# leggedrobotics/raisimLib

Measured on AMD Instinct MI355X. Metric: env-steps/sec, 4096 ANYmal-C envs flat terrain dt=0.0025, higher is better.
Workload: dtype f32

## Files before the change

include/rsb_ext.h:

```cpp
#ifndef RSB_EXT_H_
#define RSB_EXT_H_

#include "rsb.h"

#ifdef __cplusplus
extern "C" {
#endif

int rsb_set_solver_stagnation_exit(rsb_world* w, int window, double factor);
int rsb_set_solver_friction_lag(rsb_world* w, int freeze_after, int refine, double settle_tol);
int rsb_set_solver_multi_contact(rsb_world* w, int depth, int light_passes, int freeze_after, int stall_window);
int rsb_set_solver_anderson(rsb_world* w, int first_sweep, double clip);
#define RSB_SLIP_ENERGY 0
#define RSB_SLIP_COULOMB 1
int rsb_set_slip_rule(rsb_world* w, int rule);

int rsb_set_early_termination(rsb_world* w, int on);
int rsb_set_solver_warm_start(rsb_world* w, int on);

int rsb_set_lanes_per_env(rsb_world* w, int lanes);
int rsb_get_lanes_per_env(const rsb_world* w);

int rsb_set_heightmap_contacts(rsb_world* w, int per_primitive, double min_angle_deg);
int rsb_set_capsule_contacts(rsb_world* w, int on);
// ... 16 lines not shown
int rsb_model_lds_bytes(const rsb_model* m, int kmax, int self_collision, int lanes_per_env);
int rsb_model_delassus_layout(const rsb_model* m, int kmax, int self_collision, int* out4);
int rsb_model_up_quads(const rsb_model* m, int* table, int capacity);

#define RSB_SPEC_OFF 0
#define RSB_SPEC_CACHED 1
#define RSB_SPEC_COMPILE 2
int rsb_set_specialization(rsb_world* w, int mode);
int rsb_specialization_status(const rsb_world* w, long long* specialized_launches, long long* generic_launches);
const char* rsb_spec_dir(void);
int rsb_spec_compile(const char* manifest_line);
int rsb_spec_file_name(const char* manifest_line, char* out, int capacity);


int rsb_last_kernel_ms(rsb_world* w, float* ms);
int rsb_enable_timing(rsb_world* w, int on);
int rsb_set_timing_stride(rsb_world* w, int stride);
int rsb_read_kernel_ms(rsb_world* w, float* ms, int n);

int rsb_debug_select_env(rsb_world* w, int env);
int rsb_debug_read_contact_problem(rsb_world* w, int* nc, float* G, float* c, float* lam);
int rsb_debug_phase_cycles(rsb_world* w, int enable, long long* out16);
int rsb_debug_wave_profile(rsb_world* w, long long* out, int n_blocks);


#ifdef __cplusplus
}
#endif

#endif
```

raisimlib_amd/_capi.py:

```python
import ctypes as C
import os

RSB_MAX_BODIES = 64
RSB_MAX_DOF = 6 + RSB_MAX_BODIES - 1
RSB_MAX_COLLISIONS = 64
RSB_MAX_CONTACTS = 16
RSB_NAME_LEN = 48

RSB_HOST, RSB_DEVICE = 0, 1
RSB_CONTACT_SELF_A, RSB_CONTACT_SELF_B, RSB_CONTACT_SECOND, RSB_CONTACT_CAPSULE = 0x10000, 0x20000, 0x40000, 0x80000
RSB_FORCE_AND_TORQUE, RSB_PD_PLUS_FEEDFORWARD_TORQUE = 0, 1
(RSB_F_GC, RSB_F_GV, RSB_F_PTARGET, RSB_F_DTARGET, RSB_F_TAU_FF, RSB_F_CONTACT_COUNT, RSB_F_CONTACTS,
 RSB_F_FLAGS, RSB_F_GENERALIZED_FORCE) = range(9)

_B, _S = RSB_MAX_BODIES, RSB_MAX_COLLISIONS


class ModelBlob(C.Structure):
    _fields_ = [
        ("nb", C.c_int32), ("nq", C.c_int32), ("nv", C.c_int32), ("ncol", C.c_int32), ("depth", C.c_int32),
        ("fixed_base", C.c_int32),
        ("parent", C.c_int32 * _B), ("level", C.c_int32 * _B), ("jtype", C.c_int32 * _B),
        ("axis", (C.c_double * 3) * _B), ("ptree", (C.c_double * 3) * _B), ("rtree", (C.c_double * 9) * _B),
        ("mass", C.c_double * _B), ("com", (C.c_double * 3) * _B), ("inertia", (C.c_double * 6) * _B),
# ... 209 lines not shown
    "rsb_last_kernel_ms": (_I, [_VP, C.POINTER(C.c_float)]),
    "rsb_enable_timing": (_I, [_VP, _I]),
    "rsb_set_timing_stride": (_I, [_VP, _I]),
    "rsb_read_kernel_ms": (_I, [_VP, _FP, _I]),
    "rsb_control_step": (_I, [_VP, _FP, _FP, _I, _FP, _FP, _I, _FP, _I, _FP, _FP, _I]),
    "rsb_control_steps": (_I, [_VP, _I, _FP, _I, C.c_longlong, _I, _FP, C.c_longlong, _FP, _I, _FP, _I, _FP, _FP, _I, _VP, C.c_longlong]),
    "rsb_set_step_residency": (_I, [_VP, _I]),
    "rsb_step_residency_enabled": (_I, [_VP]),
    "rsb_step_residency_status": (_I, [_VP, _I]),
    "rsb_step_residency_launches": (C.c_longlong, [_VP]),
    "rsb_debug_resident_full_writes": (_I, [_VP, _I]),
    "rsb_model_lds_bytes": (_I, [_VP, _I, _I, _I]),
    "rsb_model_up_quads": (_I, [_VP, _VP, _I]),
    "rsb_model_delassus_layout": (_I, [_VP, _I, _I, _VP]),
    "rsb_set_specialization": (_I, [_VP, _I]),
    "rsb_specialization_status": (_I, [_VP, C.POINTER(C.c_longlong), C.POINTER(C.c_longlong)]),
    "rsb_spec_dir": (C.c_char_p, []),
    "rsb_spec_compile": (_I, [C.c_char_p]),
    "rsb_spec_file_name": (_I, [C.c_char_p, C.c_char_p, _I]),
    "rsb_debug_view_profile": (_I, [_VP, C.POINTER(C.c_longlong), _I]),
    "rsb_debug_select_env": (_I, [_VP, _I]),
    "rsb_debug_phase_cycles": (_I, [_VP, _I, _FP]),
    "rsb_debug_wave_profile": (_I, [_VP, _FP, _I]),
    "rsb_debug_read_contact_problem": (_I, [_VP, C.POINTER(C.c_int), _FP, _FP, _FP]),
}

_lib = None


def lib():
    global _lib
    if _lib is None:
        if not os.path.exists(LIB_PATH):
            raise RuntimeError(
                f"{LIB_PATH} is missing: build it with `python -c 'import __graft_entry__ as g; g.build()'` "
                "(hipcc --offload-arch=gfx950). raisimlib_amd has no CPU fallback.")
        L = C.CDLL(LIB_PATH, mode=C.RTLD_GLOBAL)
        for name, (res, args) in PROTOTYPES.items():
            fn = getattr(L, name)
            fn.restype, fn.argtypes = res, args
        _lib = L
    return _lib


class RsbError(RuntimeError):
    pass
# ... 7 lines not shown
```

raisimlib_amd/csrc/rsb_world.hip:

```cpp
#include <dlfcn.h>
#include <hip/hip_runtime.h>

#include <algorithm>
#include <cmath>
#include <cstdio>
#include <cstdlib>
#include <chrono>
#include <cstring>
#include <memory>
#include <string>
#include <vector>

#include "query_kernel.h"
#include "rsb.h"
#include "rsb_internal.h"
#include "step_launch.h"
#include "env_task.h"
#include "step_types.h"


#include "rsb_world.h"
#include "rsb_spec.h"

namespace rsbw {
// ... 1639 lines not shown
  if (c) std::memcpy(c, buf.data() + 1 + n3 * n3, sizeof(float) * n3);
  if (lam) std::memcpy(lam, buf.data() + 1 + n3 * n3 + n3, sizeof(float) * n3);
  return RSB_OK;
}

int rsb_debug_phase_cycles(rsb_world* w, int enable, long long* out16) {
  if (!w) return RSB_E_INVALID;
  HIP_TRY(hipSetDevice(w->device));
  const size_t nprof = 16 + 16 * (size_t)w->N;
  if (enable && !w->d_prof) { HIP_TRY(hipMalloc(&w->d_prof, nprof * sizeof(long long))); HIP_TRY(hipMemset(w->d_prof, 0, nprof * sizeof(long long))); }
  if (out16 && w->d_prof) {
    HIP_TRY(hipMemcpyAsync(out16, w->d_prof, 16 * sizeof(long long), hipMemcpyDeviceToHost, stream_of(w)));
    HIP_TRY(hipStreamSynchronize(stream_of(w)));
  }
  if (!enable && w->d_prof) { HIP_TRY(hipStreamSynchronize(stream_of(w))); HIP_TRY(hipFree(w->d_prof)); w->d_prof = nullptr; }
  return RSB_OK;
}

int rsb_debug_wave_profile(rsb_world* w, long long* out, int n_blocks) {
  if (!w || !out || !w->d_prof || n_blocks > w->N) return RSB_E_INVALID;
  HIP_TRY(hipSetDevice(w->device));
  HIP_TRY(hipMemcpyAsync(out, w->d_prof + 16, 16 * (size_t)n_blocks * sizeof(long long), hipMemcpyDeviceToHost, stream_of(w)));
  HIP_TRY(hipStreamSynchronize(stream_of(w)));
  return RSB_OK;
}

int rsb_enable_timing(rsb_world* w, int on) {
  if (!w || on < 0) return RSB_E_INVALID;
  HIP_TRY(hipSetDevice(w->device));
  for (hipEvent_t e : w->ring0) (void)hipEventDestroy(e);
  for (hipEvent_t e : w->ring1) (void)hipEventDestroy(e);
  w->ring0.clear(); w->ring1.clear(); w->ring_next = w->ring_count = 0;
  w->launch_index = 0;
  w->timing = on != 0;
  if (on > 1) {
    w->ring0.resize(on); w->ring1.resize(on);
    for (int i = 0; i < on; ++i) { HIP_TRY(hipEventCreate(&w->ring0[i])); HIP_TRY(hipEventCreate(&w->ring1[i])); }
  }
  return RSB_OK;
}
int rsb_set_timing_stride(rsb_world* w, int stride) {
  if (!w || stride < 1) return RSB_E_INVALID;
  w->timing_stride = stride; w->launch_index = 0;
  return RSB_OK;
}
int rsb_read_kernel_ms(rsb_world* w, float* ms, int n) {
// ... 23 lines not shown
```

raisimlib_amd/csrc/step_kernel.h:

```cpp
#pragma once

#include <hip/hip_runtime.h>
#include <stdint.h>

#include <type_traits>

#include "env_task.h"
#include "rsb_types.h"
#include "step_types.h"
#include "step_spec.h"
#include "step_math.h"
#include "step_terrain.h"
#include "step_slip.h"
#include "step_slip_pk.h"
#include "stage_bodies.h"

#ifndef RSB_X_RES_RING
#define RSB_X_RES_RING 0
#endif
#if defined(RSB_I_CL) && ((RSB_I_CL) & 64)
#define RSB_RESIDENT 1
#else
#define RSB_RESIDENT 0
#endif
// ... 257 lines not shown
  for (int sub = 0; sub < nsub; ++sub) {
    RSB_STAMP(0)
    RSB_ARGS(ab);
    tsq = 0.f;
#include "step_phase_tree_down.inc"
#include "step_phase_collision.inc"
#include "step_phase_tree_up.inc"
    iters_used = 0;
    float wlam[6] = {0.f, 0.f, 0.f, 0.f, 0.f, 0.f};
    if (ncw > 0) {
      RSB_ARGS(aw);
      const float erp = RSB_DIM_F32(ERP, aw.erp);
#include "step_phase_columns.inc"
#include "step_phase_delassus.inc"
#include "step_phase_solver.inc"
    } else if (has_warm) {
      for (int i = s; i < nwarm; i += LPE) WARM[i] = 0.f;
    }
    RSB_STAMP(6)

#include "step_phase_update.inc"
  }

  if (PROF && a.prof && lane == 0) { long long* P = a.prof + 16 + 16 * (long long)blk; P[8] = t_setup; P[9] = t_newt; P[10] = t_epi; P[11] = t_rule; P[12] = t_exch; P[13] = t_end; P[14] = t_start - t_entry; P[15] = t_mag; P[0] = clock64() - t_start; P[1] = t_gs; P[2] = p_iters; P[3] = p_ncw; P[4] = p_search; P[5] = p_newton; P[6] = p_solves; P[7] = t_srch; }
#if RSB_LEAN_SEAM
  if (ls_ok && cs + 1 < ncs) {
#include "step_phase_seam_lean.inc"
  } else {
    seam_refill = true;
    asm volatile("; rsb generic seam begin");
#endif
#include "step_phase_epilogue.inc"
#if RSB_LEAN_SEAM
    asm volatile("; rsb generic seam end");
  }
#endif
#if RSB_RESIDENT
  }
#endif
}

}
```

raisimlib_amd/csrc/step_phase_prologue.inc:

```
  const float* env_heights = a.heights;
  if (a.hm_index && a.terrain_type == 1) env_heights += (size_t)a.hm_index[env] * a.hm_xs * a.hm_ys;
  float rq[2], rpt[2], ru[2], rdt[2], rtf[2], ract[2] = {0.f, 0.f}, ramean[2] = {0.f, 0.f}, wrec[8];
  if constexpr (PIPE) {
    if (a.pipe_wait_on) {
      int spins = 0;
      long long t0 = 0;
      const long long t_in = a.pipe_stats ? wall_clock64() : 0;
      while (__builtin_amdgcn_readfirstlane(__hip_atomic_load(a.pipe_wait_ptr + (size_t)blk * a.pipe_stride, __ATOMIC_RELAXED, __HIP_MEMORY_SCOPE_AGENT)) - a.pipe_wait < 0) {
        if (__builtin_amdgcn_readfirstlane(__hip_atomic_load(a.pipe_err, __ATOMIC_RELAXED, __HIP_MEMORY_SCOPE_AGENT)) != 0) return;
        __builtin_amdgcn_s_sleep(8);
        if ((++spins & 255) == 0) {
          const long long now = wall_clock64();
          if (t0 == 0) t0 = now;
          else if (now - t0 > a.pipe_timeout) {
            if (lane == 0 && atomicCAS(a.pipe_err, 0, 2 ) == 0) __hip_atomic_store(a.pipe_err_host, 2, __ATOMIC_RELAXED, __HIP_MEMORY_SCOPE_SYSTEM);
            return;
          }
        }
      }
      if (a.pipe_stats && lane == 0) {
        __hip_atomic_fetch_add(a.pipe_stats, (unsigned long long)(wall_clock64() - t_in), __ATOMIC_RELAXED, __HIP_MEMORY_SCOPE_AGENT);
        if (spins > 0) __hip_atomic_fetch_add(a.pipe_stats + 1, 1ull, __ATOMIC_RELAXED, __HIP_MEMORY_SCOPE_AGENT);
      }
    }
// ... 53 lines not shown
    if (i < nv) { U[i] = (fixed_base && i < 6) ? 0.f : ru[k]; DTG[i] = rdt[k]; TF[i] = rtf[k]; }
  }
  __syncthreads();
  const bool isbody = s >= 1 && s < nb;
  const int bb = isbody ? s : 0;
  const int mylev = isbody ? (PARLV[bb] >> 8) : -1;
  const int mypar = max((PARLV[bb] & 0xff) - 1, 0);
  const int mykid = KIDX[bb];
  const int nkid0 = KIDX[0] >> 16;
  const int kid_first = KIDS[mykid & 0xffff];
  int kid0s[4];
  RSB_UNROLL for (int i = 0; i < 4; ++i) kid0s[i] = __builtin_amdgcn_readfirstlane(KIDS[i]);
  const int max_kid = RSB_DIM(MAX_KID, a.max_kid);
  if (a.warm && s < a.kmax) {
    const int col = __float_as_int(wrec[6]) - 1;
    if (col >= 0 && col < ncol) { RSB_UNROLL for (int i = 0; i < 6; ++i) WARM[6 * col + i] = wrec[i]; }
  }
  int flag = 0, iters_used = 0, nc = 0;
  int nc_real = 0;
  int nselfc = 0;
  bool dead = false;
  int nc_dead = 0;
  long long t_start = 0, t_gs = 0, t_srch = 0, t_setup = 0, t_newt = 0, t_epi = 0, t_rule = 0, t_exch = 0, t_end = 0; int p_iters = 0, p_ncw = 0, p_search = 0, p_newton = 0, p_solves = 0;
  if (PROF && a.prof) t_start = clock64();
  const bool pfine = PROF && a.prof && a.prof_fine;
  long long t_prev = 0, t_mag = 0;
  auto lap = [&](long long& acc) { if (PROF && pfine) { const long long t = clock64(); acc += t - t_prev; t_prev = t; } };
  float pbx = 0.f, pby = 0.f, pbz = 0.f;
  const float dt = a.dt;
  const int nsub = RSB_DIM(NSUB, a.nsub), kmax = RSB_DIM(KMAX, a.kmax);
  const bool has_warm = RSB_DIM(HAS_WARM, a.warm != nullptr);
  __syncthreads();

  float tsq = 0.f;
```

raisimlib_amd/csrc/step_phase_solver.inc:

```
      if (PROF && a.dbg && env == a.dbg_env && env_valid && s == 0) {
        const int n3 = 3 * nc_real;
        a.dbg[0] = (float)nc_real;
        for (int i = 0; i < n3; ++i)
          for (int j = 0; j < n3; ++j)
            a.dbg[1 + i * n3 + j] = GROWS ? G[(i / 3) * GRP + kGBlock * (j / 3) + g_block_off(i % 3, j % 3)] : !TRI ? G[i * GS + 4 * (j / 3) + (j % 3)]
                                          : (i / 3 >= j / 3 ? G[tri_off(i / 3, j / 3) + 4 * (i % 3) + (j % 3)] : G[tri_off(j / 3, i / 3) + 4 * (j % 3) + (i % 3)]);
        for (int i = 0; i < n3; ++i) a.dbg[1 + n3 * n3 + i] = CV[i];
      }
      long long t_gs0 = 0, tz0 = 0; if (PROF && a.prof) t_gs0 = clock64();
      {
        const bool isc = s < nc;
        float Gii[9], Ginv[12], v[3], lam[3] = {0.f, 0.f, 0.f};
        const float* Gmine = GROWS ? G + GRP * min(s, KMAX - 1) : G + 3 * min(s, KMAX - 1) * GS;
        RSB_UNROLL for (int q2 = 0; q2 < 9; ++q2) Gii[q2] = 0.f;
        RSB_UNROLL for (int q2 = 0; q2 < 12; ++q2) Ginv[q2] = 0.f;
        v[0] = v[1] = v[2] = 0.f;
#if RSB_FLAT_CLASS
        asm volatile("; rsb setup begin");
#endif
#if RSB_FLAT_SETUP_HEAD
        static_assert(GROWS && !TRI, "flat set-up: the row-block layout of the quadruped classes");
        const int sq = min(s, KMAX - 1);
        float fq0[5][4], fq1[5][4], fq2[5], fc4[4], fc8[4];
        {
// ... 92 lines not shown
        int wcount = 0;

        int gpos = 0, gdw = 1;
        bool light = false;
        bool multi = false;
        int sw_env = stall_window > 0 ? stall_window : -1;
        {
          static_for<0, KMAX / 4>([&](auto bc) {
            constexpr int j0 = 4 * decltype(bc)::value;
            if (j0 < ncw) {
              static_for<0, 4>([&](auto kc2) {
                constexpr int j = j0 + decltype(kc2)::value;
                const int gj = __builtin_amdgcn_update_dpp(0, gidc, 0x150 + j, 0xf, 0xf, true);
                gpos += ((gj == gidc) & (j < s)) ? 1 : 0;
              });
            }
          });
          const int gd = row_max_i32(isc ? gpos + 1 : 1);
          multi = (RSB_DIM(MULTI_DEPTH, ag.multi_depth) > 0) & (gd >= RSB_DIM(MULTI_DEPTH, ag.multi_depth));
          light = multi & (RSB_DIM(MULTI_LIGHT, ag.multi_light) != 0);
          sw_env = multi ? (RSB_DIM(MULTI_SW, ag.multi_stall_window) > 0 ? RSB_DIM(MULTI_SW, ag.multi_stall_window) : -1) : sw_env;
          gdw = env_groups_max<LPE>(gd);
        }
#ifndef RSB_X_AA8
#define RSB_X_AA8 0
#endif
        constexpr bool AA = TRI || RSB_X_AA8;
        const int aa_first = AA ? ag.anderson : 0;
        const float aa_clip = ag.anderson_clip;
        const bool aa_on = AA && multi && aa_first > 0;
        float aa_x[3] = {0.f, 0.f, 0.f}, aa_g[3] = {0.f, 0.f, 0.f}, aa_r[3] = {0.f, 0.f, 0.f};

        const int sm = min(s, KMAX - 1);
        auto coupling = [&](int k, float (&g)[3][4]) {
          if constexpr (TRI) {
            const bool tr = k > sm;
            const float* bp = G + tri_off(tr ? k : sm, tr ? sm : k);
            float t[3][4];
            RSB_UNROLL for (int rr = 0; rr < 3; ++rr) ld4(bp + 4 * rr, t[rr]);
            RSB_UNROLL for (int rr = 0; rr < 3; ++rr) {
              RSB_UNROLL for (int cc = 0; cc < 3; ++cc) g[rr][cc] = tr ? t[cc][rr] : t[rr][cc];
              g[rr][3] = 0.f;
            }
          } else if constexpr (GROWS) {
            float t[3][3];
            gblk_load(Gmine + kGBlock * k, t);
// ... 67 lines not shown
          auto one = [&](auto jc) {
            constexpr int j = decltype(jc)::value;
            float l0[3] = {x[0], x[1], x[2]};
            row_bcast_n<j, 3>(l0);
            if constexpr (PK && j < NPK) {
              float2v acc = {v[0], v[1]};
              RSB_UNROLL for (int cc = 0; cc < 3; ++cc) acc = __builtin_elementwise_fma(gp[j][cc], float2v{l0[cc], l0[cc]}, acc);
              v[0] = acc.x; v[1] = acc.y;
              v[2] = fmaf(gr[j][2], l0[2], fmaf(gr[j][1], l0[1], fmaf(gr[j][0], l0[0], v[2])));
            } else if constexpr (PK && !TRI && j < 8) {
              float gt[3][4];
              coupling(j, gt);
              RSB_UNROLL for (int rr = 0; rr < 3; ++rr)
                v[rr] = fmaf(gt[rr][2], l0[2], fmaf(gt[rr][1], l0[1], fmaf(gt[rr][0], l0[0], v[rr])));
            } else {
              const float (&gj)[3][4] = PK ? gbuf[(j / 4) & 1][j & 3] : (j < 4 ? g0[PK ? 0 : (j & 3)] : (j < 8 ? g1[PK ? 0 : (j & 3)] : (j < 12 ? g2[(KMAX > 8 && !PK ? j : 0) & 3] : gbuf[(j / 4) & 1][j & 3])));
              RSB_UNROLL for (int rr = 0; rr < 3; ++rr)
                v[rr] = fmaf(gj[rr][2], l0[2], fmaf(gj[rr][1], l0[1], fmaf(gj[rr][0], l0[0], v[rr])));
            }
            emax = fmaxf(emax, fmaxf(fabsf(l0[0]), fmaxf(fabsf(l0[1]), fabsf(l0[2]))));
          };
          static_for<0, 5>(one);
          {
            if (ncw > 5) {
              one(std::integral_constant<int, 5>{});
              if (ncw > 6) {
                one(std::integral_constant<int, 6>{});
                if (ncw > 7) {
                  one(std::integral_constant<int, 7>{});
                  static_for<2, KMAX / 4>([&](auto bc) {
                    constexpr int b = decltype(bc)::value;
                    if (4 * b < ncw) {
                      if constexpr (b >= 3 || (PK && 4 * b >= NPK)) load_block(bc);
                      static_for<4 * b, 4 * b + 4>(one);
                    }
                  });
                }
              }
            }
          }
        };

        if (has_warm) {
#if RSB_FLAT_SETUP_HEAD
          {
            const bool wok = isc && mycol < ncol;
            lam[0] = wok ? fwr[0] : 0.f; lam[1] = wok ? fwr[1] : 0.f; lam[2] = wok ? fwr[2] : 0.f;
// ... 33 lines not shown
          row_bcast_dyn_n<KMAX, 13>(c12, j);
          SlipCoef kb;
          kb.a0 = c12[0]; kb.a1 = c12[1]; kb.a2 = c12[2]; kb.n00 = c12[3]; kb.n01 = c12[4]; kb.n02 = c12[5];
          kb.n10 = c12[6]; kb.n11 = c12[7]; kb.n12 = c12[8]; kb.vn = c12[9]; kb.ls0 = c12[10]; kb.ls1 = c12[11];
          float dxy[2];
          slip_search<LPE, COUL>(kb, c12[12], section_rounds, s, el, c16, s16, DIR16, dxy);
          if (take) { sdx = dxy[0]; sdy = dxy[1]; sdst = 1; }
        };

#if !defined(RSB_X_ALIGN_SWEEP) && defined(RSB_SPECIALIZED)
#define RSB_X_ALIGN_SWEEP 0
#endif
#ifndef RSB_X_ALIGN_SWEEP
#define RSB_X_ALIGN_SWEEP 7
#endif
#ifndef RSB_X_ALIGN_SWEEP_TRI
#define RSB_X_ALIGN_SWEEP_TRI 7
#endif
        asm volatile(".p2align 5");
        static_for<0, (TRI ? RSB_X_ALIGN_SWEEP_TRI : RSB_X_ALIGN_SWEEP)>([&](auto) { asm volatile("s_nop 0"); });
#if RSB_PK_CLASS
        asm volatile("; rsb sweep begin");
#endif
        for (int it = 0; it < max_iter; ++it) {
          const bool lag = multi ? (multi_fa > 0 && it >= multi_fa) : (freeze_after > 0 && it >= freeze_after);
          float err = 0.f;
          float dl_last[3] = {0.f, 0.f, 0.f};
          if constexpr (AA) { aa_x[0] = lam[0]; aa_x[1] = lam[1]; aa_x[2] = lam[2]; }
          for (int kp = 0; kp < gdw; ++kp) {
            const bool mine = isc & !done & (gpos == kp);
            if (PROF && a.prof) ++p_solves;
            float ls[3];
#if RSB_PK_SOLVE
            const f32x2 ls01 = pk_stick(gip, f32x2{v[0], v[1]}, v[2], f32x2{lam[0], lam[1]});
            ls[0] = ls01.x; ls[1] = ls01.y;
            ls[2] = fmaf(-Ginv[8], v[2], fmaf(-Ginv[7], v[1], fmaf(-Ginv[6], v[0], lam[2])));
#else
            RSB_UNROLL for (int rr = 0; rr < 3; ++rr)
              ls[rr] = fmaf(-Ginv[3 * rr + 2], v[2], fmaf(-Ginv[3 * rr + 1], v[1], fmaf(-Ginv[3 * rr], v[0], lam[rr])));
#endif
            const float vexn = fmaf(-Gii[8], lam[2], fmaf(-Gii[7], lam[1], fmaf(-Gii[6], lam[0], v[2])));
            const bool open = vexn > 0.f;
            const bool stick = (!open) & (ls[2] >= 0.f) & (fmaf(ls[1], ls[1], ls[0] * ls[0]) <= (mu2 * ls[2]) * ls[2]);
            const bool slip = (!open) & (!stick);
            const bool usable = (sdst == 1) & (fmaf(sc.a2, sdy, fmaf(sc.a1, sdx, sc.a0)) >= kDenFreeze * sc.a0);
            const bool keep = lag & usable;
            const bool refr = isc & !done & (light ? (kp == 0) : (gpos == kp));
            bool need = refr & slip & !keep;
            const bool lost = mine & slip & !refr & !usable;
            lap(t_rule);
#ifdef RSB_X_NO_NEWTON
            if (false) {
#else
            if (__any(need | lost)) {
#endif
              SlipCoef kc;
              kc = sc;
#if RSB_PK_SOLVE
              SlipCoefPk kp;
              pk_coef(kp, sc.a0, sc.a1, sc.a2, gcp[2], mg1, mg2, pk_vex(gcp, f32x2{v[0], v[1]}, f32x2{lam[0], lam[1]}, lam[2]), vexn, ls01);
              kc = slip_unpack(kp);
#else
              {
                const float vex0 = v[0] - (Gii[0] * lam[0] + Gii[1] * lam[1] + Gii[2] * lam[2]);
                const float vex1 = v[1] - (Gii[3] * lam[0] + Gii[4] * lam[1] + Gii[5] * lam[2]);
                kc.n00 = sc.a0 * vex0 - vexn * Gii[2]; kc.n01 = sc.a1 * vex0 - vexn * sc.n01; kc.n02 = sc.a2 * vex0 - vexn * sc.n02;
                kc.n10 = sc.a0 * vex1 - vexn * Gii[5]; kc.n11 = sc.a1 * vex1 - vexn * sc.n11; kc.n12 = sc.a2 * vex1 - vexn * sc.n12;
                kc.vn = vexn; kc.ls0 = ls[0]; kc.ls1 = ls[1];
              }
#endif
              if (PROF && a.prof) ++p_newton;
              float nx, ny, dstep;
#if RSB_PK_SOLVE
              bool ok = slip_newton_pk(kp, mu, sdx, sdy, nx, ny, dstep) & need & (sdst != 0) & (refine != 0);
#else
              bool ok = slip_newton<COUL>(kc, mu, sdx, sdy, nx, ny, dstep) & need & (sdst != 0) & (refine != 0);
#endif
#ifdef RSB_X_STAMP_BASIN
              lap(t_newt);
#endif
#ifdef RSB_X_NO_BASIN
              if (false) {
#else
              if (it == 0 && !COUL) {
#endif
                const bool chk = ok & (sdst == 3);
                if (__any(chk)) {
                  float ebest;
#ifndef RSB_X_SERIAL_BASIN
                  if (ncw <= 4) {
                    const int row = lane & ~15, q = lane & 3;
                    const int from_owner = (row | ((lane >> 2) & 3)) << 2, from_quad = (row | ((lane & 3) << 2)) << 2;
                    float c13[13] = {kc.a0, kc.a1, kc.a2, kc.n00, kc.n01, kc.n02, kc.n10, kc.n11, kc.n12, kc.vn, kc.ls0, kc.ls1, mu};
                    RSB_UNROLL for (int i = 0; i < 13; ++i) c13[i] = __int_as_float(__builtin_amdgcn_ds_bpermute(from_owner, __float_as_int(c13[i])));
                    SlipCoef kq;
                    kq.a0 = c13[0]; kq.a1 = c13[1]; kq.a2 = c13[2]; kq.n00 = c13[3]; kq.n01 = c13[4]; kq.n02 = c13[5];
                    kq.n10 = c13[6]; kq.n11 = c13[7]; kq.n12 = c13[8]; kq.vn = c13[9]; kq.ls0 = c13[10]; kq.ls1 = c13[11];
                    float e = __int_as_float(0x7f800000);
                    const bool swp = (q & 1) != 0;
                    const unsigned sgx = ((q + 1) & 2) ? 0x80000000u : 0u, sgy = (q & 2) ? 0x80000000u : 0u;
                    RSB_UNROLL for (int i = 0; i < 4; ++i) {
                      const float x = __uint_as_float(__float_as_uint(swp ? kSin16[i] : kCos16[i]) ^ sgx);
                      const float y = __uint_as_float(__float_as_uint(swp ? kCos16[i] : kSin16[i]) ^ sgy);
                      e = fminf(e, slip_E(kq, c13[12], x, y));
                    }
                    e = fminf(e, __int_as_float(__builtin_amdgcn_update_dpp(0, __float_as_int(e), 0xB1, 0xf, 0xf, true)));
                    e = fminf(e, __int_as_float(__builtin_amdgcn_update_dpp(0, __float_as_int(e), 0x4E, 0xf, 0xf, true)));
                    ebest = __int_as_float(__builtin_amdgcn_ds_bpermute(from_quad, __float_as_int(e)));
#ifdef RSB_X_BASIN_VERIFY
                    {
                      float e2 = slip_E(kc, mu, 1.0f, 0.0f);
                      RSB_UNROLL for (int i = 1; i < 16; ++i) e2 = fminf(e2, slip_E(kc, mu, kCos16[i], kSin16[i]));
                      if (chk && __float_as_int(e2) != __float_as_int(ebest)) flag |= 16;
                    }
#endif
                  } else
#endif
                  {
                    SlipCoef ks = kc;
#ifndef RSB_X_SERIAL_BASIN
                    asm volatile("" : "+v"(ks.a0), "+v"(ks.a1), "+v"(ks.a2));
#endif
                    ebest = slip_E(ks, mu, 1.0f, 0.0f);
                    RSB_UNROLL for (int i = 1; i < 16; ++i) ebest = fminf(ebest, slip_E(ks, mu, kCos16[i], kSin16[i]));
                  }
                  ok = ok & !(chk & !(slip_E(kc, mu, nx, ny) <= ebest));
                }
              }
#ifdef RSB_X_STAMP_BASIN
              lap(t_mag);
#endif
              sdx = ok ? nx : sdx; sdy = ok ? ny : sdy; sdst = ok ? 1 : sdst;
              need = (need & !ok) | lost;
              if (__any(need)) {
                for (int j = 0; j < ncw; ++j)
                  if (__any(need && s == j)) search_row(j, kc, need && s == j);
              }
              lap(t_newt);
            }
            const float den = fmaf(sc.a2, sdy, fmaf(sc.a1, sdx, sc.a0));
            const float lnn = -vexn * __builtin_amdgcn_rcpf(fmaxf(den, kDenMin * sc.a0));
            const float ltn = mu * lnn;
            float ln[3];
            float dl[3];
#if RSB_PK_SOLVE
            {
              const f32x2 lt = pk_splat(ltn) * f32x2{sdx, sdy};
              ln[0] = slip ? lt.x : (stick ? ls[0] : 0.f);
              ln[1] = slip ? lt.y : (stick ? ls[1] : 0.f);
              ln[2] = slip ? lnn : (stick ? ls[2] : 0.f);
              const f32x2 l01 = f32x2{lam[0], lam[1]}, df = pk_splat(alpha) * (f32x2{ln[0], ln[1]} - l01);
              dl[0] = mine ? df.x : 0.f; dl[1] = mine ? df.y : 0.f;
              dl[2] = mine ? alpha * (ln[2] - lam[2]) : 0.f;
              const f32x2 ln01 = l01 + f32x2{dl[0], dl[1]};
              lam[0] = ln01.x; lam[1] = ln01.y; lam[2] += dl[2];
            }
#else
            ln[0] = slip ? ltn * sdx : (stick ? ls[0] : 0.f);
            ln[1] = slip ? ltn * sdy : (stick ? ls[1] : 0.f);
            ln[2] = slip ? lnn : (stick ? ls[2] : 0.f);
            RSB_UNROLL for (int rr = 0; rr < 3; ++rr) {
              dl[rr] = mine ? alpha * (ln[rr] - lam[rr]) : 0.f;
              lam[rr] += dl[rr];
            }
#endif
            lap(t_mag);
            if constexpr (AA) {
              if (kp + 1 < gdw) exchange(dl, err);
              else { dl_last[0] = dl[0]; dl_last[1] = dl[1]; dl_last[2] = dl[2]; }
            } else {
              exchange(dl, err);
            }
            lap(t_exch);
          }
          if constexpr (AA)
            err = fmaxf(err, row_max_f32(fmaxf(fabsf(dl_last[0]), fmaxf(fabsf(dl_last[1]), fabsf(dl_last[2])))));
          if (it == 0) sdst = (sdst == 3) ? 0 : sdst;
          const float scale = row_max_f32(isc ? lam[2] : 0.f);
          {
            const bool live = !done;
            iters_used += live ? 1 : 0;
            alpha = fmaxf(alpha * alpha_decay, alpha_min);
            const float denom = scale + kLambdaFloor;
            const bool conv_now = live & (err <= threshold * denom);
            const float rel = err * __builtin_amdgcn_rcpf(denom);
            const bool cont = live & !conv_now;
            const bool better = cont & (rel < best_rel);
            best_rel = better ? rel : best_rel;
            RSB_UNROLL for (int rr = 0; rr < 3; ++rr) lam_best[rr] = better ? lam[rr] : lam_best[rr];
            best_cur = cont ? fminf(best_cur, rel) : best_cur;
            wcount += cont ? 1 : 0;
            const bool wfull = cont & (wcount == sw_env);
            const bool stalled = wfull & (best_cur > stall_factor * best_prev);
            best_prev = wfull ? best_cur : best_prev;
            best_cur = wfull ? 3e38f : best_cur;
            wcount = wfull ? 0 : wcount;
            converged |= conv_now;
            done |= conv_now | stalled;
          }
          lap(t_epi);
          if (!__any(!done)) break;
          if constexpr (AA) {
            if (__any(aa_on & !done)) {
              float rr[3], num = 0.f, den = 0.f;
              RSB_UNROLL for (int q2 = 0; q2 < 3; ++q2) {
                rr[q2] = lam[q2] - aa_x[q2];
                const float dr = rr[q2] - aa_r[q2];
                num = fmaf(rr[q2], dr, num); den = fmaf(dr, dr, den);
              }
              num = row_sum_f32(isc ? num : 0.f); den = row_sum_f32(isc ? den : 0.f);
              if constexpr (LPE > 16) {
                num = __shfl(num, (lane & ~(LPE - 1)) | (lane & 15)); den = __shfl(den, (lane & ~(LPE - 1)) | (lane & 15));
              }
              const bool use = aa_on & !done & (it >= 1) & (it + 1 >= aa_first) & (den > 1e-30f);
              float gam = use ? num / den : 0.f;
              gam = (fabsf(gam) <= aa_clip) ? gam : 0.f;
              float xn[3], dl[3];
              RSB_UNROLL for (int q2 = 0; q2 < 3; ++q2) { xn[q2] = fmaf(-gam, lam[q2] - aa_g[q2], lam[q2]); aa_g[q2] = lam[q2]; aa_r[q2] = rr[q2]; }
              const float t2 = fmaf(xn[1], xn[1], xn[0] * xn[0]), lim = mu * xn[2];
              const float sh = (t2 > lim * lim) ? lim * __builtin_amdgcn_rsqf(t2) : 1.f;
              const bool off = xn[2] <= 0.f;
              xn[0] = off ? 0.f : xn[0] * sh; xn[1] = off ? 0.f : xn[1] * sh; xn[2] = off ? 0.f : xn[2];
              const bool app = isc & (gam != 0.f);
              RSB_UNROLL for (int q2 = 0; q2 < 3; ++q2) { dl[q2] = app ? xn[q2] - lam[q2] : 0.f; lam[q2] += dl[q2]; dl_last[q2] += dl[q2]; }
// ... 142 lines not shown
```

raisimlib_amd/csrc/step_slip_pk.h:

```cpp
#pragma once

#include "step_slip.h"

#define RSB_PK_NO_CONTRACT _Pragma("clang fp contract(off)")

namespace rsbk {

typedef float f32x2 __attribute__((ext_vector_type(2)));

__device__ __forceinline__ f32x2 pk_splat(float a) { return f32x2{a, a}; }
__device__ __forceinline__ f32x2 pk_fma(f32x2 a, f32x2 b, f32x2 c) { return __builtin_elementwise_fma(a, b, c); }
__device__ __forceinline__ f32x2 pk_swap(f32x2 a) { return f32x2{a.y, a.x}; }

struct SlipCoefPk { float a0, a1, a2, vn; f32x2 n0, n1, n2, ls; };

__device__ __forceinline__ SlipCoef slip_unpack(const SlipCoefPk& k) {
  SlipCoef s;
  s.a0 = k.a0; s.a1 = k.a1; s.a2 = k.a2; s.vn = k.vn;
  s.n00 = k.n0.x; s.n10 = k.n0.y; s.n01 = k.n1.x; s.n11 = k.n1.y; s.n02 = k.n2.x; s.n12 = k.n2.y;
  s.ls0 = k.ls.x; s.ls1 = k.ls.y;
  return s;
}

__device__ __forceinline__ f32x2 pk_stick(const f32x2 (&gi)[3], f32x2 v01, float v2, f32x2 lam01) { RSB_PK_NO_CONTRACT
// ... 24 lines not shown

__device__ __forceinline__ float slip_newton_step_pk(const SlipCoefPk& k, float x0, float y0, float den, float& hp) { RSB_PK_NO_CONTRACT
  const f32x2 xx = pk_splat(x0), yy = pk_splat(y0), ym = f32x2{-y0, y0};
  const float mdp = __builtin_fmaf(k.a2, x0, -(k.a1 * y0));
  const f32x2 N = pk_fma(yy, k.n2, pk_fma(xx, k.n1, k.n0));
  const f32x2 dN = pk_fma(xx, k.n2, -(yy * k.n1));
  const f32x2 PQ = pk_fma(xx, pk_swap(N), ym * N);
  const f32x2 AB = pk_fma(xx, pk_swap(dN), ym * dN);
  const float h = __builtin_fmaf(den, PQ.x, -(mdp * PQ.y));
  hp = __builtin_fmaf(-mdp, AB.y, __builtin_fmaf(den, AB.x, -(k.a0 * PQ.y)));
  return -h * __builtin_amdgcn_rcpf(hp);
}

__device__ __forceinline__ f32x2 slip_rotate_pk(f32x2 d0, float d) { RSB_PK_NO_CONTRACT
  const float d2 = d * d;
  const float c = __builtin_fmaf(-d2, __builtin_fmaf(-d2, 1.0f / 24.0f, 0.5f), 1.0f);
  const float t = __builtin_fmaf(-d2, __builtin_fmaf(-d2, 1.0f / 120.0f, 1.0f / 6.0f), 1.0f);
  const f32x2 sn = f32x2{-d, d} * pk_splat(t);
  const f32x2 xy = pk_fma(d0, pk_splat(c), pk_swap(d0) * sn);
  const float inv = __builtin_amdgcn_rsqf(__builtin_fmaf(xy.x, xy.x, xy.y * xy.y));
  return xy * pk_splat(inv);
}

__device__ __forceinline__ bool slip_newton_pk(const SlipCoefPk& k, float mu, float x0, float y0, float& x1, float& y1, float& step) { RSB_PK_NO_CONTRACT
  const float den0 = pk_den(k, x0, y0);
  float hp;
  const float d = slip_newton_step_pk(k, x0, y0, den0, hp);
  const f32x2 xy = slip_rotate_pk(f32x2{x0, y0}, d);
  const float den1 = pk_den(k, xy.x, xy.y);
  bool ok = (den0 > kDenNewton * k.a0) && (hp > 0.f) && (fabsf(d) <= 0.25f) && (den1 > kDenNewton * k.a0);
  if (__any(ok && fabsf(d) > 0.02f)) ok = ok && (fabsf(d) <= 0.02f || slip_E_pk(k, mu, xy.x, xy.y, den1) <= slip_E_pk(k, mu, x0, y0, den0));
  x1 = xy.x; y1 = xy.y; step = d;
  return ok;
}

}
```

raisimlib_amd/csrc/step_spec.h:

```cpp
#pragma once

#define RSB_SPEC_FIELDS(X)                                                                                                              \
  X(NB, a.nb) X(NQ, a.nq) X(NV, a.nv) X(DEPTH, a.depth) X(NCOL, a.ncol) X(MAX_KID, a.max_kid) X(FIXED_BASE, (a.fixed_base != 0))      \
  X(N_SELF, a.n_self) X(NSUB, a.nsub) X(KMAX, a.kmax) X(HAS_WARM, (a.warm != nullptr)) X(TERRAIN, a.terrain_type)                      \
  X(EARLY_TERM, (a.early_term != 0)) X(SECTION_ROUNDS, a.section_rounds) X(STALL_WINDOW, a.stall_window) X(FREEZE_AFTER, a.freeze_after) \
  X(REFINE, a.refine) X(MULTI_FA, a.multi_freeze_after) X(MULTI_DEPTH, a.multi_depth) X(MULTI_LIGHT, a.multi_light)                    \
  X(MULTI_SW, a.multi_stall_window) X(CHAIN, (a.chain != 0)) X(MODEL_PITCH, a.L.model_pitch) \
  X(UP_QUADS, (a.chain == 2)) \
  X(MU, rsbk::spec_bits(a.mu)) X(ERP, rsbk::spec_bits(a.erp)) X(ALPHA_INIT, rsbk::spec_bits(a.alpha_init)) X(ALPHA_MIN, rsbk::spec_bits(a.alpha_min)) \
  X(ALPHA_DECAY, rsbk::spec_bits(a.alpha_decay)) X(THRESHOLD, rsbk::spec_bits(a.threshold)) X(STALL_FACTOR, rsbk::spec_bits(a.stall_factor)) \
  X(MAX_ITER, a.max_iter)

#ifdef RSB_SPECIALIZED
#define RSB_DIM(NAME, expr) (RSB_SPEC_##NAME)
#else
#define RSB_DIM(NAME, expr) (expr)
#endif

namespace rsbk {
constexpr int spec_bits(float f) { return __builtin_bit_cast(int, f); }
constexpr float spec_f32(int bits) { return __builtin_bit_cast(float, bits); }
}
#if defined(RSB_SPECIALIZED) && !defined(RSB_X_NO_SPEC_CONSTS)
#define RSB_SPEC_CONSTS 1
// ... 89 lines not shown
#if RSB_FLAT_SETUP && RSB_FLAT_SCATTER && !defined(RSB_X_NO_FLAT_SETUP_END)
#define RSB_FLAT_SETUP_END 1
#else
#define RSB_FLAT_SETUP_END 0
#endif

#if RSB_FLAT_SETUP && (RSB_I_KMAX) == 8 && RSB_SPEC_UP_QUADS && !defined(RSB_X_NO_FLAT_DELASSUS)
#define RSB_FLAT_DELASSUS 1
#else
#define RSB_FLAT_DELASSUS 0
#endif

#if defined(RSB_SPECIALIZED) && defined(RSB_I_LPE) && (RSB_I_LPE) == 16 && (RSB_I_KMAX) <= 8 && !((RSB_I_CL) & 32)
#define RSB_PK_CLASS 1
#else
#define RSB_PK_CLASS 0
#endif
#if RSB_PK_CLASS && !defined(RSB_X_NO_PK_SOLVE)
#define RSB_PK_SOLVE 1
#else
#define RSB_PK_SOLVE 0
#endif

namespace rsbk {
#define RSB_SPEC_COUNT_ONE(NAME, expr) +1
constexpr int kSpecFields = 0 RSB_SPEC_FIELDS(RSB_SPEC_COUNT_ONE);
#undef RSB_SPEC_COUNT_ONE
}
```

raisimlib_amd/world.py:

```python
import ctypes as C
import os

import numpy as np

from . import _capi
from ._capi import (RSB_DEVICE, RSB_F_GENERALIZED_FORCE, RSB_HOST, RSB_MAX_CONTACTS, Contact, ModelBlob, check, lib)

RSC_DIR = os.path.join(os.path.dirname(os.path.abspath(__file__)), "rsc")

CONTACT_DTYPE = np.dtype([("position", "f4", 3), ("normal", "f4", 3), ("impulse", "f4", 3), ("depth", "f4"),
                          ("body", "i4"), ("collision", "i4")])
assert CONTACT_DTYPE.itemsize == C.sizeof(Contact)


def rsc_path(name):
    return os.path.join(RSC_DIR, name)


class Model:

    def __init__(self, urdf_path=None, urdf_string=None, blob=None, sample_spacing=0.0):
        L = lib()
        h = C.c_void_p()
        if urdf_path is not None:
# ... 970 lines not shown

    def debug_contact_problem(self):
        K = RSB_MAX_CONTACTS
        G = np.zeros(9 * K * K, np.float32)
        c = np.zeros(3 * K, np.float32)
        lam = np.zeros(3 * K, np.float32)
        nc = C.c_int()
        check(self.L.rsb_debug_read_contact_problem(self.handle, C.byref(nc), _hp(G), _hp(c), _hp(lam)),
              "rsb_debug_read_contact_problem")
        n3 = 3 * nc.value
        return nc.value, G[:n3 * n3].reshape(n3, n3).copy(), c[:n3].copy(), lam[:n3].copy()

    def debug_phase_cycles(self, enable=True, read=True):
        out = np.zeros(16, np.int64)
        check(self.L.rsb_debug_phase_cycles(self.handle, 1 if enable else 0, _hp(out) if read else None),
              "rsb_debug_phase_cycles")
        return out

    def debug_wave_profile(self):
        nb = (self.N * self.lanes_per_env() + 63) // 64
        out = np.zeros((nb, 16), np.int64)
        check(self.L.rsb_debug_wave_profile(self.handle, _hp(out), nb), "rsb_debug_wave_profile")
        return out
```

Before: 397.4 million.

## Restructure solver sweep loop with scalar control and wave-uniform rare-path skip

Splits the packed slip Newton into a core step and an energy check, and skips the energy check, basin test and search block whenever no lane in the wave takes a rare case. Fast lanes accept the core Newton result directly. The sweep and iteration loops are rewritten as do/while and for(;;) loops with the counters kept in scalar registers (readfirstlane, ballot-based exit) to cut branch and loop-control overhead. It also adds optional per-wave counters for sweep control paths and a debug readout API. The risk is extra register pressure and a subtle change in which lanes accept the Newton step without the energy test.

```diff
diff --git a/include/rsb_ext.h b/include/rsb_ext.h
--- a/include/rsb_ext.h
+++ b/include/rsb_ext.h
@@ -62,6 +62,7 @@
 int rsb_debug_read_contact_problem(rsb_world* w, int* nc, float* G, float* c, float* lam);
 int rsb_debug_phase_cycles(rsb_world* w, int enable, long long* out16);
 int rsb_debug_wave_profile(rsb_world* w, long long* out, int n_blocks);
+int rsb_debug_wave_sweep_control(rsb_world* w, long long* out, int n_blocks);
 
 
 #ifdef __cplusplus
diff --git a/raisimlib_amd/_capi.py b/raisimlib_amd/_capi.py
--- a/raisimlib_amd/_capi.py
+++ b/raisimlib_amd/_capi.py
@@ -255,6 +255,7 @@
     "rsb_debug_select_env": (_I, [_VP, _I]),
     "rsb_debug_phase_cycles": (_I, [_VP, _I, _FP]),
     "rsb_debug_wave_profile": (_I, [_VP, _FP, _I]),
+    "rsb_debug_wave_sweep_control": (_I, [_VP, _FP, _I]),
     "rsb_debug_read_contact_problem": (_I, [_VP, C.POINTER(C.c_int), _FP, _FP, _FP]),
 }
 
diff --git a/raisimlib_amd/csrc/rsb_world.hip b/raisimlib_amd/csrc/rsb_world.hip
--- a/raisimlib_amd/csrc/rsb_world.hip
+++ b/raisimlib_amd/csrc/rsb_world.hip
@@ -1685,6 +1685,19 @@
   HIP_TRY(hipSetDevice(w->device));
   HIP_TRY(hipMemcpyAsync(out, w->d_prof + 16, 16 * (size_t)n_blocks * sizeof(long long), hipMemcpyDeviceToHost, stream_of(w)));
   HIP_TRY(hipStreamSynchronize(stream_of(w)));
+  for (int b = 0; b < n_blocks; ++b)
+    for (int i = 2; i < 8; ++i) out[16 * (size_t)b + i] &= 0xffffffffll;
+  return RSB_OK;
+}
+
+int rsb_debug_wave_sweep_control(rsb_world* w, long long* out, int n_blocks) {
+  if (!w || !out || !w->d_prof || n_blocks > w->N) return RSB_E_INVALID;
+  HIP_TRY(hipSetDevice(w->device));
+  std::vector<long long> raw(16 * (size_t)n_blocks);
+  HIP_TRY(hipMemcpyAsync(raw.data(), w->d_prof + 16, raw.size() * sizeof(long long), hipMemcpyDeviceToHost, stream_of(w)));
+  HIP_TRY(hipStreamSynchronize(stream_of(w)));
+  for (int b = 0; b < n_blocks; ++b)
+    for (int i = 0; i < 12; ++i) out[12 * (size_t)b + i] = (raw[16 * (size_t)b + 2 + i / 2] >> (32 + 16 * (i & 1))) & 0xffff;
   return RSB_OK;
 }
 
diff --git a/raisimlib_amd/csrc/step_kernel.h b/raisimlib_amd/csrc/step_kernel.h
--- a/raisimlib_amd/csrc/step_kernel.h
+++ b/raisimlib_amd/csrc/step_kernel.h
@@ -303,7 +303,8 @@
 #include "step_phase_update.inc"
   }
 
-  if (PROF && a.prof && lane == 0) { long long* P = a.prof + 16 + 16 * (long long)blk; P[8] = t_setup; P[9] = t_newt; P[10] = t_epi; P[11] = t_rule; P[12] = t_exch; P[13] = t_end; P[14] = t_start - t_entry; P[15] = t_mag; P[0] = clock64() - t_start; P[1] = t_gs; P[2] = p_iters; P[3] = p_ncw; P[4] = p_search; P[5] = p_newton; P[6] = p_solves; P[7] = t_srch; }
+  if (PROF && a.prof && lane == 0) { long long* P = a.prof + 16 + 16 * (long long)blk; P[8] = t_setup; P[9] = t_newt; P[10] = t_epi; P[11] = t_rule; P[12] = t_exch; P[13] = t_end; P[14] = t_start - t_entry; P[15] = t_mag; P[0] = clock64() - t_start; P[1] = t_gs; P[2] = p_iters; P[3] = p_ncw; P[4] = p_search; P[5] = p_newton; P[6] = p_solves; P[7] = t_srch;
+    RSB_UNROLL for (int i = 0; i < 12; ++i) P[2 + i / 2] |= (long long)min(p_ctl[i], 0xffff) << (32 + 16 * (i & 1)); }
 #if RSB_LEAN_SEAM
   if (ls_ok && cs + 1 < ncs) {
 #include "step_phase_seam_lean.inc"
diff --git a/raisimlib_amd/csrc/step_phase_prologue.inc b/raisimlib_amd/csrc/step_phase_prologue.inc
--- a/raisimlib_amd/csrc/step_phase_prologue.inc
+++ b/raisimlib_amd/csrc/step_phase_prologue.inc
@@ -99,7 +99,14 @@
   bool dead = false;
   int nc_dead = 0;
   long long t_start = 0, t_gs = 0, t_srch = 0, t_setup = 0, t_newt = 0, t_epi = 0, t_rule = 0, t_exch = 0, t_end = 0; int p_iters = 0, p_ncw = 0, p_search = 0, p_newton = 0, p_solves = 0;
+  enum { kCtlNewtonFirst = 0, kCtlRareFirst, kCtlRareLater, kCtlEnergyFirst, kCtlEnergyLater, kCtlBasinQuad, kCtlBasinSerial, kCtlSearchFirst, kCtlSearchLater, kCtlNoneFirst, kCtlNoneLater, kCtlRefused };
+  int p_ctl[12] = {0, 0, 0, 0, 0, 0, 0, 0, 0, 0, 0, 0};
   if (PROF && a.prof) t_start = clock64();
+#ifdef RSB_X_SWEEP_COUNTERS
+  const bool pctl = PROF && a.prof;
+#else
+  constexpr bool pctl = false;
+#endif
   const bool pfine = PROF && a.prof && a.prof_fine;
   long long t_prev = 0, t_mag = 0;
   auto lap = [&](long long& acc) { if (PROF && pfine) { const long long t = clock64(); acc += t - t_prev; t_prev = t; } };
diff --git a/raisimlib_amd/csrc/step_phase_solver.inc b/raisimlib_amd/csrc/step_phase_solver.inc
--- a/raisimlib_amd/csrc/step_phase_solver.inc
+++ b/raisimlib_amd/csrc/step_phase_solver.inc
@@ -138,6 +138,10 @@
           sw_env = multi ? (RSB_DIM(MULTI_SW, ag.multi_stall_window) > 0 ? RSB_DIM(MULTI_SW, ag.multi_stall_window) : -1) : sw_env;
           gdw = env_groups_max<LPE>(gd);
         }
+#if RSB_SWEEP_LOOP
+        gdw = __builtin_amdgcn_readfirstlane(gdw);
+        asm volatile("" : "+s"(gdw));
+#endif
 #ifndef RSB_X_AA8
 #define RSB_X_AA8 0
 #endif
@@ -251,7 +255,11 @@
           };
           static_for<0, 5>(one);
           {
+#if RSB_SWEEP_LOOP
+            if (__builtin_expect(ncw > 5, 0)) {
+#else
             if (ncw > 5) {
+#endif
               one(std::integral_constant<int, 5>{});
               if (ncw > 6) {
                 one(std::integral_constant<int, 6>{});
@@ -331,13 +339,31 @@
 #if RSB_PK_CLASS
         asm volatile("; rsb sweep begin");
 #endif
+#if RSB_SWEEP_LOOP
+        static_assert(!(TRI || RSB_X_AA8), "sweep control: the Anderson step sits behind the exit test of the loop it replaces");
+        int it = 0, kp = 0;
+        float err = 0.f;
+        bool act = isc & !done;
+        asm volatile("" : "+s"(kp), "+v"(err));
+        if (max_iter > 0) for (;;) {
+#else
         for (int it = 0; it < max_iter; ++it) {
+#endif
+#if !RSB_SWEEP_LOOP
           const bool lag = multi ? (multi_fa > 0 && it >= multi_fa) : (freeze_after > 0 && it >= freeze_after);
           float err = 0.f;
+#endif
           float dl_last[3] = {0.f, 0.f, 0.f};
           if constexpr (AA) { aa_x[0] = lam[0]; aa_x[1] = lam[1]; aa_x[2] = lam[2]; }
+#if RSB_SWEEP_LOOP
+          do {
+            asm volatile("; rsb sweep control end" : "+s"(kp), "+s"(it));
+            const bool lag = multi ? (multi_fa > 0 && it >= multi_fa) : (freeze_after > 0 && it >= freeze_after);
+            const bool mine = act & (gpos == kp);
+#else
           for (int kp = 0; kp < gdw; ++kp) {
             const bool mine = isc & !done & (gpos == kp);
+#endif
             if (PROF && a.prof) ++p_solves;
             float ls[3];
 #if RSB_PK_SOLVE
@@ -354,7 +380,11 @@
             const bool slip = (!open) & (!stick);
             const bool usable = (sdst == 1) & (fmaf(sc.a2, sdy, fmaf(sc.a1, sdx, sc.a0)) >= kDenFreeze * sc.a0);
             const bool keep = lag & usable;
+#if RSB_SWEEP_LOOP
+            const bool refr = act & (light ? (kp == 0) : (gpos == kp));
+#else
             const bool refr = isc & !done & (light ? (kp == 0) : (gpos == kp));
+#endif
             bool need = refr & slip & !keep;
             const bool lost = mine & slip & !refr & !usable;
             lap(t_rule);
@@ -379,9 +409,31 @@
               }
 #endif
               if (PROF && a.prof) ++p_newton;
+              bool p_cont = false;
               float nx, ny, dstep;
 #if RSB_PK_SOLVE
-              bool ok = slip_newton_pk(kp, mu, sdx, sdy, nx, ny, dstep) & need & (sdst != 0) & (refine != 0);
+              f32x2 nxy;
+              float den0, den1;
+              const bool okcore = slip_newton_core_pk(kp, sdx, sdy, nxy, dstep, den0, den1);
+              nx = nxy.x; ny = nxy.y;
+              const bool okc = okcore & need & (sdst != 0) & (refine != 0);
+#ifdef RSB_X_NO_BASIN
+              const bool rare_l = (okc & (fabsf(dstep) > 0.02f)) | (need & !okc) | lost;
+#else
+              const bool rare_l = (okc & (fabsf(dstep) > 0.02f)) | ((it == 0) & okc & (sdst == 3)) | (need & !okc) | lost;
+#endif
+              if (PROF && pctl) {
+                if (it == 0) ++p_ctl[kCtlNewtonFirst];
+                const bool pr = __any(rare_l);
+                if (pr) ++p_ctl[it == 0 ? kCtlRareFirst : kCtlRareLater];
+                if ((RSB_SWEEP_RARE ? pr : true) && __any(okcore & (fabsf(dstep) > 0.02f))) { ++p_ctl[it == 0 ? kCtlEnergyFirst : kCtlEnergyLater]; p_cont = true; }
+              }
+#if RSB_SWEEP_RARE
+              bool okf = okc;
+              const bool p_rare = __any(rare_l);
+              if (__builtin_expect(p_rare, 1)) {
+#endif
+              bool ok = slip_newton_energy_pk(kp, mu, sdx, sdy, nxy, dstep, den0, den1, okcore) & need & (sdst != 0) & (refine != 0);
 #else
               bool ok = slip_newton<COUL>(kc, mu, sdx, sdy, nx, ny, dstep) & need & (sdst != 0) & (refine != 0);
 #endif
@@ -395,6 +447,7 @@
 #endif
                 const bool chk = ok & (sdst == 3);
                 if (__any(chk)) {
+                  if (PROF && pctl) { ++p_ctl[ncw <= 4 ? kCtlBasinQuad : kCtlBasinSerial]; p_cont = true; }
                   float ebest;
 #ifndef RSB_X_SERIAL_BASIN
                   if (ncw <= 4) {
@@ -439,13 +492,31 @@
 #ifdef RSB_X_STAMP_BASIN
               lap(t_mag);
 #endif
+              if (PROF && pctl) { if (__any(need & (sdst != 0) & !ok)) ++p_ctl[kCtlRefused]; }
               sdx = ok ? nx : sdx; sdy = ok ? ny : sdy; sdst = ok ? 1 : sdst;
               need = (need & !ok) | lost;
               if (__any(need)) {
+                if (PROF && pctl) { ++p_ctl[it == 0 ? kCtlSearchFirst : kCtlSearchLater]; p_cont = true; }
                 for (int j = 0; j < ncw; ++j)
                   if (__any(need && s == j)) search_row(j, kc, need && s == j);
               }
+              if (PROF && pctl) { if (!p_cont) ++p_ctl[it == 0 ? kCtlNoneFirst : kCtlNoneLater]; }
               lap(t_newt);
+#if RSB_SWEEP_RARE
+                okf = false;
+              }
+              asm volatile("; rsb refresh fast begin" : "+v"(sdx), "+v"(sdy), "+v"(sdst));
+              sdx = okf ? nx : sdx; sdy = okf ? ny : sdy; sdst = okf ? 1 : sdst;
+              asm volatile("; rsb refresh fast end" : "+v"(sdx), "+v"(sdy), "+v"(sdst));
+              if (PROF && pctl) { if (!p_rare) ++p_ctl[it == 0 ? kCtlNoneFirst : kCtlNoneLater]; }
+              if (PROF && pfine) { if (!p_rare) {
+#ifdef RSB_X_STAMP_BASIN
+                lap(t_newt);
+                lap(t_mag);
+#endif
+                lap(t_newt);
+              } }
+#endif
             }
             const float den = fmaf(sc.a2, sdy, fmaf(sc.a1, sdx, sc.a0));
             const float lnn = -vexn * __builtin_amdgcn_rcpf(fmaxf(den, kDenMin * sc.a0));
@@ -481,7 +552,14 @@
               exchange(dl, err);
             }
             lap(t_exch);
-          }
+#if RSB_SWEEP_LOOP
+            asm volatile("; rsb sweep control begin");
+            ++kp;
+            asm volatile("" : "+s"(kp));
+          } while (__builtin_expect(kp < gdw, 0));
+#else
+          }
+#endif
           if constexpr (AA)
             err = fmaxf(err, row_max_f32(fmaxf(fabsf(dl_last[0]), fmaxf(fabsf(dl_last[1]), fabsf(dl_last[2])))));
           if (it == 0) sdst = (sdst == 3) ? 0 : sdst;
@@ -506,9 +584,24 @@
             wcount = wfull ? 0 : wcount;
             converged |= conv_now;
             done |= conv_now | stalled;
+#if RSB_SWEEP_LOOP
+            act = act & !(conv_now | stalled);
+#endif
           }
           lap(t_epi);
+#if RSB_SWEEP_LOOP
+          ++it;
+          kp = 0; err = 0.f;
+          asm volatile("" : "+s"(it), "+s"(kp), "+v"(err));
+          {
+            unsigned long long live = __builtin_amdgcn_ballot_w64(!done);
+            live = (it < max_iter) ? live : 0ull;
+            asm volatile("" : "+s"(live));
+            if (live == 0ull) break;
+          }
+#else
           if (!__any(!done)) break;
+#endif
           if constexpr (AA) {
             if (__any(aa_on & !done)) {
               float rr[3], num = 0.f, den = 0.f;
diff --git a/raisimlib_amd/csrc/step_slip_pk.h b/raisimlib_amd/csrc/step_slip_pk.h
--- a/raisimlib_amd/csrc/step_slip_pk.h
+++ b/raisimlib_amd/csrc/step_slip_pk.h
@@ -70,14 +70,23 @@
   return xy * pk_splat(inv);
 }
 
+__device__ __forceinline__ bool slip_newton_core_pk(const SlipCoefPk& k, float x0, float y0, f32x2& xy, float& d, float& den0, float& den1) { RSB_PK_NO_CONTRACT
+  den0 = pk_den(k, x0, y0);
+  float hp;
+  d = slip_newton_step_pk(k, x0, y0, den0, hp);
+  xy = slip_rotate_pk(f32x2{x0, y0}, d);
+  den1 = pk_den(k, xy.x, xy.y);
+  return (den0 > kDenNewton * k.a0) && (hp > 0.f) && (fabsf(d) <= 0.25f) && (den1 > kDenNewton * k.a0);
+}
+__device__ __forceinline__ bool slip_newton_energy_pk(const SlipCoefPk& k, float mu, float x0, float y0, f32x2 xy, float d, float den0, float den1, bool ok) { RSB_PK_NO_CONTRACT
+  if (__any(ok && fabsf(d) > 0.02f)) ok = ok && (fabsf(d) <= 0.02f || slip_E_pk(k, mu, xy.x, xy.y, den1) <= slip_E_pk(k, mu, x0, y0, den0));
+  return ok;
+}
 __device__ __forceinline__ bool slip_newton_pk(const SlipCoefPk& k, float mu, float x0, float y0, float& x1, float& y1, float& step) { RSB_PK_NO_CONTRACT
-  const float den0 = pk_den(k, x0, y0);
-  float hp;
-  const float d = slip_newton_step_pk(k, x0, y0, den0, hp);
-  const f32x2 xy = slip_rotate_pk(f32x2{x0, y0}, d);
-  const float den1 = pk_den(k, xy.x, xy.y);
-  bool ok = (den0 > kDenNewton * k.a0) && (hp > 0.f) && (fabsf(d) <= 0.25f) && (den1 > kDenNewton * k.a0);
-  if (__any(ok && fabsf(d) > 0.02f)) ok = ok && (fabsf(d) <= 0.02f || slip_E_pk(k, mu, xy.x, xy.y, den1) <= slip_E_pk(k, mu, x0, y0, den0));
+  f32x2 xy;
+  float d, den0, den1;
+  const bool core = slip_newton_core_pk(k, x0, y0, xy, d, den0, den1);
+  const bool ok = slip_newton_energy_pk(k, mu, x0, y0, xy, d, den0, den1, core);
   x1 = xy.x; y1 = xy.y; step = d;
   return ok;
 }
diff --git a/raisimlib_amd/csrc/step_spec.h b/raisimlib_amd/csrc/step_spec.h
--- a/raisimlib_amd/csrc/step_spec.h
+++ b/raisimlib_amd/csrc/step_spec.h
@@ -135,6 +135,22 @@
 #define RSB_PK_SOLVE 0
 #endif
 
+#if RSB_PK_SOLVE && !defined(RSB_X_NO_SWEEP_CONTROL)
+#define RSB_SWEEP_CONTROL 1
+#else
+#define RSB_SWEEP_CONTROL 0
+#endif
+#if RSB_SWEEP_CONTROL && !defined(RSB_X_NO_SWEEP_CONTROL_RARE)
+#define RSB_SWEEP_RARE 1
+#else
+#define RSB_SWEEP_RARE 0
+#endif
+#if RSB_SWEEP_CONTROL && !defined(RSB_X_NO_SWEEP_CONTROL_LOOP)
+#define RSB_SWEEP_LOOP 1
+#else
+#define RSB_SWEEP_LOOP 0
+#endif
+
 namespace rsbk {
 #define RSB_SPEC_COUNT_ONE(NAME, expr) +1
 constexpr int kSpecFields = 0 RSB_SPEC_FIELDS(RSB_SPEC_COUNT_ONE);
diff --git a/raisimlib_amd/world.py b/raisimlib_amd/world.py
--- a/raisimlib_amd/world.py
+++ b/raisimlib_amd/world.py
@@ -1016,3 +1016,9 @@
         out = np.zeros((nb, 16), np.int64)
         check(self.L.rsb_debug_wave_profile(self.handle, _hp(out), nb), "rsb_debug_wave_profile")
         return out
+
+    def debug_wave_sweep_control(self):
+        nb = (self.N * self.lanes_per_env() + 63) // 64
+        out = np.zeros((nb, 12), np.int64)
+        check(self.L.rsb_debug_wave_sweep_control(self.handle, _hp(out), nb), "rsb_debug_wave_sweep_control")
+        return out
```

Result: faster. 403.0 million (median of 6 runs) (+1.4%).
